# linchaobao/EPPM

Hardware: AMD Instinct MI355X
Metric: Mflow-vectors/sec (higher is better)
Workload: dtype f32; 1 GPU; single 1024x436 Sintel-shape synthetic pair per step, full 3-level pyramid, patch_r=9, default defs.h parameters; 1 rank(s), independent pairs; inputs: RGBA planes resident in HBM before the timed region; outputs: interleaved float2 flow left in HBM (the PCIe-inclusive window of the reference API -- host RGB in, host u/v out -- is `host_boundary`, with --full); inputs=device-resident RGBA, outputs=device-resident float2 flow, pairs_in_flight_per_gpu=24, pairs_per_launch=8, contexts_in_flight=3, width=1024, height=436

## Files before the change

### eppm_amd/_lib.py

```python
import ctypes as C
import os

from .build import lib_path


class EppmError(RuntimeError):
    pass


class CParams(C.Structure):
    _fields_ = [("patch_r", C.c_int), ("num_iter", C.c_int), ("search_range", C.c_int), ("num_guess", C.c_int),
                ("seg_len", C.c_int), ("wmf_iters", C.c_int), ("seed", C.c_ulonglong), ("propagation", C.c_int),
                ("levels", C.c_int)]


class CTrackParams(C.Structure):
    _fields_ = [("spacing", C.c_int), ("min_eig", C.c_int64), ("fb_alpha", C.c_float), ("fb_beta", C.c_float), ("mb_alpha", C.c_float),
                ("mb_beta", C.c_float), ("capacity", C.c_int)]


class CTrackCounts(C.Structure):
    _fields_ = [("live", C.c_int), ("ended", C.c_int), ("seeded", C.c_int), ("dropped", C.c_int), ("frame", C.c_int), ("next_id", C.c_int)]

    def as_dict(self):
        return {k: int(getattr(self, k)) for k, _ in self._fields_}


_lib = None

SYMBOLS = [
    "eppm_default_params", "eppm_create", "eppm_create_batch", "eppm_batch_size", "eppm_batch_set_images", "eppm_batch_set_images_device",
    "eppm_batch_compute", "eppm_batch_compute_device", "eppm_batch_compute_end", "eppm_batch_get_plane", "eppm_destroy", "eppm_set_stream", "eppm_set_images", "eppm_set_images_device",
    "eppm_compute", "eppm_compute_begin", "eppm_compute_end", "eppm_compute_device", "eppm_synchronize", "eppm_num_levels", "eppm_level_dims", "eppm_get_plane",
    "eppm_stage_times", "eppm_clear_stage_times", "eppm_enable_stage_timing", "eppm_last_error", "eppm_version",
    "eppm_device_count", "eppm_set_device", "eppm_malloc_device", "eppm_malloc_pitched", "eppm_free_device",
    "eppm_memcpy_h2d", "eppm_memcpy_d2h", "eppm_memcpy2d_h2d", "eppm_memcpy2d_d2h", "eppm_memset_device",
    "eppm_device_synchronize", "eppm_device_mem_info", "eppm_device_pci_bus_id", "eppm_bind_thread_to_device", "eppm_release_cached_memory", "eppm_set_launcher_stream", "eppm_set_launcher_params", "eppm_launcher_status",
    "baoCudaPatchMatchMultiscalePrepare", "baoCudaCensusTransform", "baoCudaPatchMatch", "baoCudaLeftRightCheck",
    "baoCudaOutlierRemoval", "baoCudaWeightedMedianFilter", "baoCudaFillHole", "baoCudaNNF2Flow", "baoCudaBLF_C2F",
    "baoCudaBLFCostFilterRefine", "baoCudaFlowSmoothing", "eppm_flow_to_color", "eppm_compute_color",
    "eppm_pm_rng_create", "eppm_pm_rng_reset", "eppm_pm_rng_destroy", "eppm_pm_rng_block_states", "eppm_pm_gen_rand_field",
    "eppm_pm_cost_field", "eppm_pm_seg_propagate", "eppm_pm_jump_propagate", "eppm_pm_parallel_propagate", "eppm_pm_random_search", "eppm_gauss_filter_rgba", "eppm_resize_rgba",
    "eppm_resize_flow",
    "eppm_host_register", "eppm_host_unregister", "eppm_host_is_registered", "eppm_host_alloc", "eppm_host_free",
    "eppm_compute_begin_into", "eppm_batch_compute_begin_into",
    "eppm_load_ppm", "eppm_ppm_size", "eppm_save_flo", "eppm_load_flo", "eppm_flo_size", "eppm_flow_error",
    "eppm_flow_error_border", "eppm_flow_error_percentage", "eppm_flow_cutoff", "eppm_flow_to_color_host",
    "eppm_compute_bidirectional", "eppm_compute_bidirectional_device", "eppm_batch_compute_bidirectional", "eppm_set_occlusion_params",
    "eppm_fb_occlusion", "eppm_fb_occlusion_host",
    "eppm_interpolate", "eppm_interpolate_device", "eppm_batch_interpolate", "eppm_interpolate_frames", "eppm_interpolate_host",
    "eppm_track_default_params", "eppm_track_capacity", "eppm_tracker_create", "eppm_tracker_destroy", "eppm_track_step",
    "eppm_track_step_frames", "eppm_tracker_get", "eppm_tracker_get_ended", "eppm_tracker_set", "eppm_track_step_host", "eppm_track_seeds_host",
]


TEST_SYMBOLS = ["eppm_test_set_option", "eppm_probe_c2f_window", "eppm_probe_fast_exp", "eppm_probe_div_const", "eppm_probe_delta_table"]

_variant = None


def select_library(variant):
    global _variant
    if _lib is not None and variant != _variant:
        raise EppmError("select_library: a library is loaded already")
    _variant = variant


def lib():
    global _lib
    if _lib is None:
        path = lib_path(_variant)
        if not os.path.exists(path):
            raise EppmError(f"{path} is missing: run eppm_amd.build() (hipcc --offload-arch=gfx950); there is no CPU fallback")
        L = C.CDLL(path)
        L.eppm_last_error.restype = C.c_char_p
        L.eppm_version.restype = C.c_char_p
        _lib = L
    return _lib


def check(status, what=""):
    if status != 0:
        raise EppmError(f"{what}: status {status}: {lib().eppm_last_error().decode()}")


def check_launcher(what=""):
    check(lib().eppm_launcher_status(), what)
```

### eppm_amd/csrc/context.cpp

```cpp
#include "api_internal.h"
#include "interp.h"

using namespace eppm;


struct StageEv { const char* name; hipEvent_t a, b; };

struct eppm_ctx {
    int device = 0;
    hipStream_t stream = nullptr;
    bool own_stream = false;
    int opt_sweep_spec = -1, opt_no_split = 0;
    eppm_params prm;
    int h = 0, w = 0, nl = 0;
    int npairs = 1, n_active = 1;
    char* slab = nullptr;
    size_t stride = 0;
    int H[kMaxLevels], W[kMaxLevels];
    size_t ipitch[kMaxLevels], cpitch[kMaxLevels];
    uint32_t *raw1 = nullptr, *raw2 = nullptr;
    size_t raw_pitch = 0;
    uint32_t *img1[kMaxLevels] = {}, *img2[kMaxLevels] = {}, *tmpu[kMaxLevels] = {};
    uint8_t *cen1[kMaxLevels] = {}, *cen2[kMaxLevels] = {};
    void *pk1[kMaxLevels] = {}, *pk2[kMaxLevels] = {};
// ... 139 lines not shown
}

static int ctx_alloc(eppm_ctx* c)
{
    const int h = c->h, w = c->w;
    size_t off = 0;
    auto take = [&](size_t bytes) { const size_t o = off; off = (off + bytes + 255) & ~(size_t)255; return o; };
    auto pitch_of = [](size_t row_bytes) { return (row_bytes + 255) & ~(size_t)255; };
    struct Fix { void** dst; size_t off; };
    std::vector<Fix> fix;
    auto plane = [&](void** dst, size_t bytes) { fix.push_back(Fix{dst, take(bytes)}); };
    c->raw_pitch = pitch_of((size_t)w * 4);
    plane((void**)&c->raw1, c->raw_pitch * h);
    plane((void**)&c->raw2, c->raw_pitch * h);
    for (int i = 0; i < c->nl; i++) {
        c->ipitch[i] = pitch_of((size_t)c->W[i] * 4);
        c->cpitch[i] = pitch_of((size_t)c->W[i]);
        const size_t n = (size_t)c->W[i] * c->H[i];
        plane((void**)&c->img1[i], c->ipitch[i] * c->H[i]);
        plane((void**)&c->img2[i], c->ipitch[i] * c->H[i]);
        plane((void**)&c->tmpu[i], c->ipitch[i] * c->H[i]);
        plane(&c->pk1[i], n * 16);
        plane(&c->pk2[i], n * 16);
        plane((void**)&c->pc1[i], n * 4);
        plane((void**)&c->pc2[i], n * 4);
        plane((void**)&c->cen1[i], c->cpitch[i] * c->H[i]);
        plane((void**)&c->cen2[i], c->cpitch[i] * c->H[i]);
        plane((void**)&c->flow[i], n * 8);
        plane((void**)&c->flow_tmp[i], n * 8);
        if (i < c->nl - 1 && c2f_refine_wants_split(c->W[i], c->H[i], c->prm.patch_r, 1, c->opt_no_split != 0)) plane((void**)&c->c2f_cost9[i], n * 36 * 4);
    }
    const int L = c->nl - 1;
    const size_t n2 = (size_t)c->W[L] * c->H[L];
#ifdef EPPM_TOL
    c->pp_pad = (c->prm.patch_r + 2) & ~1;
    c->pp_pitch = parity_pitch(c->W[L], c->pp_pad);
    plane((void**)&c->pp1, (size_t)2 * c->H[L] * c->pp_pitch * 4);
    plane((void**)&c->pp2, (size_t)2 * c->H[L] * c->pp_pitch * 4);
#endif
    plane((void**)&c->nnf1, n2 * 4);
    plane((void**)&c->nnf2, n2 * 4);
    plane((void**)&c->nnf_tmp, n2 * 4);
    plane((void**)&c->nnf_tmp2, n2 * 4);
    plane((void**)&c->cost1, n2 * 4);
    plane((void**)&c->cost2, n2 * 4);
    plane((void**)&c->spec1, n2 * 4 * 4);
    plane((void**)&c->spec2, n2 * 4 * 4);
    plane((void**)&c->scand1, n2 * 4 * 4);
    plane((void**)&c->scand2, n2 * 4 * 4);
    plane((void**)&c->wl1, pm_worklist_words(c->W[L], c->H[L], c->prm.seg_len) * 4);
    plane((void**)&c->wl2, pm_worklist_words(c->W[L], c->H[L], c->prm.seg_len) * 4);
    plane((void**)&c->seed1, n2 * 4 * 4);
    plane((void**)&c->seed2, n2 * 4 * 4);
    plane((void**)&c->wmf_ws, wmf_workspace_words(c->W[L], c->H[L], c->prm.wmf_iters) * 4);
    plane((void**)&c->d_rgb, (size_t)h * w * 3 * 2);
    plane((void**)&c->d_color, (size_t)h * w * 4);
    plane((void**)&c->d_uv, (size_t)h * w * 8);
    CHK(rng_create(&c->rng, c->W[L], c->H[L], c->prm, false));
    const size_t rng_bytes = (size_t)c->rng->gx * c->rng->gy * 64 * 6 * 4;
    for (int k = 0; k < 2; k++)
        for (int q = 0; q < 2; q++) plane((void**)&c->rng->work[k][q], rng_bytes);
    c->stride = (off + 4095) & ~(size_t)4095;
    c->slab_bytes = c->stride * c->npairs;
    {
        const hipError_t e = cache_alloc((void**)&c->slab, c->slab_bytes, false, c->device);
        if (e != hipSuccess) { (void)hipGetLastError(); return set_err(EPPM_ERR_HIP, "hipMalloc of %zu bytes (%d slab(s)) failed: %s", c->slab_bytes, c->npairs, hipGetErrorString(e)); }
    }
    for (const Fix& f : fix) *f.dst = c->slab + f.off;
    CHK(shared_luts(c->device, c->prm.patch_r, &c->lut_pm, &c->lut_wmf, &c->lut_blf));
    c->out_u.assign(c->npairs, nullptr);
    c->out_v.assign(c->npairs, nullptr);
    return EPPM_OK;
// ... 744 lines not shown
        pitch = (size_t)w * esz;
        pstride = c->bwd_stride;
    }
    else return set_err(EPPM_ERR_ARG, "eppm_get_plane: unknown plane '%s' at level %d", name, level);
    if (dst_bytes < (size_t)w * h * esz) return set_err(EPPM_ERR_ARG, "eppm_get_plane: dst too small");
    HIPCHK(hipMemcpy2D(dst, (size_t)w * esz, (const char*)src + (size_t)pair * pstride, pitch, (size_t)w * esz, h, hipMemcpyDeviceToHost));
    return EPPM_OK;
}

extern "C" int eppm_get_plane(eppm_ctx* c, const char* name, int level, void* dst, size_t dst_bytes)
{
    return eppm_batch_get_plane(c, 0, name, level, dst, dst_bytes);
}

extern "C" int eppm_compute_color(eppm_ctx* c, uint8_t* rgb, size_t row_stride, float max_disp_x, float max_disp_y)
{
    if (!c || !rgb) return set_err(EPPM_ERR_ARG, "eppm_compute_color: NULL argument");
    if (!c->have_flow) return set_err(EPPM_ERR_STATE, "eppm_compute_color: no flow computed yet");
    if (row_stride < (size_t)c->w * 3) return set_err(EPPM_ERR_ARG, "eppm_compute_color: row_stride %zu < 3*w", row_stride);
    HIPCHK(hipSetDevice(c->device));
    const size_t n = (size_t)c->h * c->w;
    if (!c->h_color) HIPCHK(hipHostMalloc((void**)&c->h_color, n * 4, hipHostMallocDefault));
    launch_flow_to_color(c->d_color, c->flow[0], c->h, c->w, max_disp_x, max_disp_y, c->stream);
    HIPCHK(hipMemcpyAsync(c->h_color, c->d_color, n * 4, hipMemcpyDeviceToHost, c->stream));
    HIPCHK(hipStreamSynchronize(c->stream));
    for (int y = 0; y < c->h; y++)
        for (int x = 0; x < c->w; x++) {
            const uint32_t p = c->h_color[(size_t)y * c->w + x];
            uint8_t* o = rgb + (size_t)y * row_stride + (size_t)x * 3;
            o[0] = (uint8_t)(p & 0xff); o[1] = (uint8_t)((p >> 8) & 0xff); o[2] = (uint8_t)((p >> 16) & 0xff);
        }
    return EPPM_OK;
}
```

### eppm_amd/csrc/eppm_device.cuh

```cuda
#pragma once

#include <hip/hip_runtime.h>
#include <stdint.h>
#include <float.h>
#include <type_traits>

#include "eppm_internal.h"

namespace eppm {

template <class T>
__device__ __forceinline__ T* pair_ptr(T* p, size_t stride, unsigned pair)
{
    using Byte = typename std::conditional<std::is_const<T>::value, const char, char>::type;
    return reinterpret_cast<T*>(reinterpret_cast<Byte*>(p) + stride * pair);
}
template <class T>
__device__ __forceinline__ T* pair_ptr_opt(T* p, size_t stride, unsigned pair)
{
    return p ? pair_ptr(p, stride, pair) : p;
}

constexpr float kLambdaAd2 = 0.1f * 0.1f;
constexpr float kPmSigR2 = 0.1f * 0.1f;
// ... 34 lines not shown
__device__ __forceinline__ float unorm8(float c) { constexpr DivConst d = make_div_const(255.0f); return div_const(c, d); }

struct rgbf { float x, y, z; };

__device__ __forceinline__ rgbf unpack_rgb(uint32_t p)
{
    rgbf r;
    r.x = unorm8((float)(p & 0xffu));
    r.y = unorm8((float)((p >> 8) & 0xffu));
    r.z = unorm8((float)((p >> 16) & 0xffu));
    return r;
}

__device__ __forceinline__ int iclamp(int v, int lo, int hi) { return min(max(v, lo), hi); }
__device__ __forceinline__ int med3i(int v, int lo, int hi)
{
    int r;
    asm("v_med3_i32 %0, %1, %2, %3" : "=v"(r) : "v"(v), "v"(lo), "v"(hi));
    return r;
}

__device__ __forceinline__ float max_abs_diff(const rgbf a, const rgbf b)
{
    return fmaxf(fmaxf(fabsf(a.x - b.x), fabsf(a.y - b.y)), fabsf(a.z - b.z));
}

struct Planes {
    const float4* pk1;
    const float4* pk2;
    int w, h;
    int pitch;
};

#ifndef EPPM_TOL
#ifndef EPPM_CENSUS_POPCNT
#define EPPM_CENSUS_POPCNT 1
#endif
__device__ __forceinline__ float4 make_texel(uint32_t rgba, uint32_t census)
{
    const rgbf c = unpack_rgb(rgba);
    return make_float4(c.x, c.y, c.z, __uint_as_float(EPPM_CENSUS_POPCNT ? (census & 0xffu) * 0x01010101u : (census & 0xffu) << 2));
}
__device__ __forceinline__ float census_cost(const float* __restrict__ cnx, uint32_t w1, uint32_t w2)
{
    return *reinterpret_cast<const float*>(reinterpret_cast<const char*>(cnx) + (EPPM_CENSUS_POPCNT ? (uint32_t)__builtin_popcount(w1 ^ w2) : (w1 ^ w2)));
}
#else
constexpr unsigned kTolScale = 4u;
__device__ __forceinline__ float4 make_texel(uint32_t rgba, uint32_t census)
{
    return make_float4(__uint_as_float((rgba & 0xffu) * kTolScale), __uint_as_float(((rgba >> 8) & 0xffu) * kTolScale),
                       __uint_as_float(((rgba >> 16) & 0xffu) * kTolScale), __uint_as_float((census & 0xffu) * 0x01010101u));
}
#endif
__device__ __forceinline__ float one_minus_fast_exp(float x) { return 1 - fast_exp(x); }

struct DeltaTab {
    int t1[256];
    float t2[kDeltaSlots];
};
#ifndef EPPM_DELTA_PATCH
#define EPPM_DELTA_PATCH 1
#endif
#ifndef EPPM_DELTA_BLF
#define EPPM_DELTA_BLF 1
#endif
typedef const __attribute__((address_space(3))) float lds_cfloat;
typedef const __attribute__((address_space(3))) int lds_cint;
__device__ __forceinline__ uint32_t lds_addr(const void* p) { return (uint32_t)(uintptr_t)(const __attribute__((address_space(3))) void*)p; }
__device__ __forceinline__ float delta_lookup(const DeltaTab& D, float d)
{
    const uint32_t a1 = __float_as_uint(__builtin_fmaf(d, __uint_as_float(1020u), __uint_as_float(lds_addr(D.t1))));
    const uint32_t a2 = (__float_as_uint(d) << 2) + (uint32_t)*reinterpret_cast<lds_cint*>(a1);
    return *reinterpret_cast<lds_cfloat*>(a2);
}
__device__ __forceinline__ float delta_lookup_off(const DeltaTab& D, float d)
{
    const uint32_t o1 = __float_as_uint(d * __uint_as_float(1020u));
// ... 70 lines not shown
    float cn[16];
};
__device__ __forceinline__ uint32_t linf_off(const rgbf a, const rgbf b) { return __float_as_uint(max_abs_diff(a, b)); }
__device__ __forceinline__ float tol_at(const float* __restrict__ t, uint32_t byte_off)
{
    return *reinterpret_cast<const float*>(reinterpret_cast<const char*>(t) + byte_off);
}
__device__ __forceinline__ float tol_cost(const TolTables& T, const rgbf p1, const rgbf p2, uint32_t w1, uint32_t w2)
{
    return tol_at(T.td, linf_off(p1, p2)) + tol_at(T.cn, (uint32_t)__builtin_popcount(w1 ^ w2));
}
constexpr float kTolExpC = (float)(1.4426950408889634 / (255.0 * 255.0 * (double)kPmSigR2) / (double)(kTolScale * kTolScale));
constexpr float kTolWeightBias = 24.0f;
__device__ __forceinline__ float tol_exp_arg(uint32_t off4k, float lsrc)
{
    const float kf = __uint_as_float(off4k) * 0x1p100f;
    return __builtin_fmaf(kf * kf, -kTolExpC * 0x1p98f, lsrc);
}
__device__ __forceinline__ rgbf tol_scale_centre(const rgbf c) { return rgbf{c.x * 0x1p100f, c.y * 0x1p100f, c.z * 0x1p100f}; }
__device__ __forceinline__ float tol_exp_arg_scaled(const rgbf cs, const rgbf p, float lsrc)
{
    const float kf = fmaxf(fmaxf(fabsf(__builtin_fmaf(p.x, 0x1p100f, -cs.x)), fabsf(__builtin_fmaf(p.y, 0x1p100f, -cs.y))), fabsf(__builtin_fmaf(p.z, 0x1p100f, -cs.z)));
    return __builtin_fmaf(kf * kf, -kTolExpC * 0x1p98f, lsrc);
}
__device__ __forceinline__ float4 unpack_texel(uint32_t w, uint32_t two)
{
    uint32_t r, g, b;
    asm("v_lshlrev_b32_sdwa %0, %1, %2 dst_sel:DWORD dst_unused:UNUSED_PAD src0_sel:DWORD src1_sel:BYTE_0" : "=v"(r) : "v"(two), "v"(w));
    asm("v_lshlrev_b32_sdwa %0, %1, %2 dst_sel:DWORD dst_unused:UNUSED_PAD src0_sel:DWORD src1_sel:BYTE_1" : "=v"(g) : "v"(two), "v"(w));
    asm("v_lshlrev_b32_sdwa %0, %1, %2 dst_sel:DWORD dst_unused:UNUSED_PAD src0_sel:DWORD src1_sel:BYTE_2" : "=v"(b) : "v"(two), "v"(w));
    static_assert(kTolScale == 4u, "the shift above");
    return make_float4(__uint_as_float(r), __uint_as_float(g), __uint_as_float(b), __uint_as_float(__builtin_amdgcn_perm(w, w, 0x03030303u)));
}
typedef uint32_t u32x4 __attribute__((ext_vector_type(4)));
typedef uint32_t u32x2 __attribute__((ext_vector_type(2)));
__device__ __forceinline__ void patch_terms(const float4 q1, const float4 q2, const rgbf c1, const rgbf c2, float gsp,
                                            const TolTables& T, float& cost_term, float& weight_term)
{
    const rgbf p1 = texel_rgb(q1);
    const rgbf p2 = texel_rgb(q2);
    cost_term = tol_cost(T, p1, p2, __float_as_uint(q1.w), __float_as_uint(q2.w));
    weight_term = (tol_at(T.ta, linf_off(c1, p1)) * gsp) * tol_at(T.ta, linf_off(c2, p2));
}
__device__ __forceinline__ void patch_accum(float& cost_sum, float& weight_sum, float cost_term, float weight_term)
{
    cost_sum = __builtin_fmaf(cost_term, weight_term, cost_sum);
    weight_sum += weight_term;
}
#endif

template <class TAB>
__device__ __forceinline__ void patch_sample(const Planes& P, const rgbf c1, const rgbf c2, int sx1, int sy1, int sx2,
                                             int sy2, float gsp, const TAB& cnx, float& cost_term,
                                             float& weight_term)
{
    const float4 q1 = tex_px(P.pk1, P.pitch, P.w, P.h, sx1, sy1);
    const float4 q2 = tex_px(P.pk2, P.pitch, P.w, P.h, sx2, sy2);
    patch_terms(q1, q2, c1, c2, gsp, cnx, cost_term, weight_term);
}

__host__ __device__ constexpr int tol_chunk(int R) { return R == 17 ? 6 : (R + 2) / 2; }
struct PatchSum {
    float cs = 0.0f, ws = 0.0f;
#ifdef EPPM_TOL
    float cc = 0.0f, cw = 0.0f;
    __device__ __forceinline__ void add(float cost_term, float weight_term) { patch_accum(cc, cw, cost_term, weight_term); }
    __device__ __forceinline__ void flush() { cs += cc; ws += cw; cc = 0.0f; cw = 0.0f; }
#else
// ... 154 lines not shown
```

### eppm_amd/csrc/eppm_internal.h

```cpp
#pragma once

#include <hip/hip_runtime.h>
#include <stddef.h>
#include <stdint.h>

#include "../../include/eppm.h"

namespace eppm {

constexpr int kMaxLevels = 8;
constexpr int kNumLevels = 3;
constexpr int kBlock = 16;
constexpr int kMaxS = 32;
constexpr int kWmfRadius = 4;
constexpr int kBlfRadius = 10;
constexpr int kDeltaSlots = 800;

struct Batch {
    int n;
    size_t stride;
};
constexpr Batch kOnePair = {1, 0};

struct PlanesH {
// ... 35 lines not shown
    int32_t* scand = nullptr;
    uint32_t* wl = nullptr;
    int16_t* seed = nullptr;
    uint32_t* rng_work;
    uint32_t* rng_work_next;
};
struct PmBatch {
    PmProblem p[2];
    int n;
    int cpitch, npitch;
    int npairs = 1;
    size_t stride = 0;
    size_t cache_plane = 0;
    int wl_units = 0;
    int sweep_seq = 0;
    size_t seed_plane = 0;
    int merged_it = 0;
    int seg_len = 0, nseg_row = 0, nseg_col = 0;
};
int pm_worklist_units(int w, int h, int seg_len);
inline size_t pm_worklist_words(int w, int h, int seg_len) { return 16 + 10 * (size_t)pm_worklist_units(w, h, seg_len); }
struct PmRngDev {
    const uint32_t* init_tab;
    const uint32_t* iter_tab;
    const uint32_t* skip_mat;
    uint32_t skip_weyl;
    int per_lane;
    int gx, gy;
    const int16_t* rand_tab = nullptr;
};
void launch_pm_rand_table(const PmRngDev& rng, uint32_t* work, int16_t* tab, int G, hipStream_t s);
void launch_pm_init_field(const PmBatch& b, const PmRngDev& rng, hipStream_t s);
void launch_pm_cost_field(const PmBatch& b, const float* lut, int R, hipStream_t s);
bool launch_pm_sweep(PmBatch& b, const float* lut, int R, int seg_len, int dir, hipStream_t s, bool speculative = false);
bool launch_pm_sweeps_merged(PmBatch& b, const float* lut, int R, int seg_len, int iteration, hipStream_t s);
void launch_pm_jump(const PmBatch& b, const float* lut, int R, int step, hipStream_t s);
void launch_pm_neighbor(const PmBatch& b, const float* lut, int R, hipStream_t s);
void launch_pm_random_search(const PmBatch& b, const PmRngDev& rng, const float* lut, int R, int search_range, int num_guess,
                             hipStream_t s);

void launch_lr_check(int16_t* nnf1, float* cost1, const int16_t* nnf2, int w, int h, int cost_pitch, int nnf_pitch, hipStream_t s, Batch bt = kOnePair);
void launch_outlier(int16_t* nnf_out, float* cost, const int16_t* nnf_in, int w, int h, int cost_pitch, int nnf_pitch, hipStream_t s, Batch bt = kOnePair);
size_t wmf_workspace_words(int w, int h, int num_iter);
int16_t* launch_wmf(int16_t* buf_a, int16_t* buf_b, const uint32_t* img, int ipitch, int w, int h, int nnf_pitch,
                    const float* wmf_lut, int num_iter, int only_occlusion, uint32_t* ws, hipStream_t s, Batch bt = kOnePair);
void launch_fill_holes(int16_t* nnf_out, const int16_t* nnf_in, const uint32_t* img, int ipitch, int w, int h, int nnf_pitch,
                       hipStream_t s, Batch bt = kOnePair);
void launch_nnf2flow(float* flow, int flow_pitch, const int16_t* nnf, int nnf_pitch, int w, int h, hipStream_t s, Batch bt = kOnePair);

void launch_resize_flow(float* out, int outH, int outW, const float* in, int h, int w, float ratio, float post_scale, hipStream_t s, Batch bt = kOnePair);
void launch_mul_scalar(float* flow, float scale, int h, int w, hipStream_t s);
bool c2f_refine_wants_split(int w, int h, int R, int npairs = 1, bool no_split = false);
bool c2f_window_span(int R, int* span_x, int* span_y);
void launch_c2f_refine(const PlanesH& P, float* flow, const float* lut, int R, float* cost9, hipStream_t s, Batch bt = kOnePair, bool no_split = false);
void launch_flow_blf(float* out, const float* in, const uint32_t* img, int ipitch, int w, int h, int flow_pitch,
                     const float* blf_lut, hipStream_t s, Batch bt = kOnePair);

void launch_split_flow(float* uv, const float* flow, int n, hipStream_t s, Batch bt = kOnePair);

void launch_fb_occlusion(uint8_t* occ1, uint8_t* occ2, const float* fwd, size_t fwd_stride, const float* bwd, size_t bwd_stride, int h, int w,
                         float alpha, float beta, int npairs, int ndir, hipStream_t s);

constexpr int kInterpChunk = 4;
struct InterpArgs {
    const uint8_t* img1;
    const uint8_t* img2;
// ... 26 lines not shown
    struct {
        int spacing;
        long long min_eig;
        float fb_alpha, fb_beta, mb_alpha, mb_beta;
    } p;
    int cap, ncells, ncx;
    float* npos;
    uint8_t* stat;
    TrackRec* ended;
    int32_t* ended_reason;
    uint8_t* cov;
    uint8_t* flags;
    int32_t *blk_s, *blk_e;
    int32_t* blk_c;
    int32_t* cnt;
};
struct TrackIn {
    const uint8_t* img1;
    const uint8_t* img2;
    size_t pitch;
    const float* fwd;
    const float* bwd;
    int h, w;
};
void launch_track_seed0(const TrackDev& d, const TrackIn& in, TrackRec* cur, hipStream_t s);
void launch_track_advance(const TrackDev& d, const TrackIn& in, const TrackRec* cur, hipStream_t s);
void launch_track_seed(const TrackDev& d, const TrackIn& in, hipStream_t s);
void launch_track_compact(const TrackDev& d, const TrackIn& in, const TrackRec* cur, TrackRec* next, hipStream_t s);

void launch_flow_to_color(uint32_t* rgba, const float* flow, int h, int w, float max_disp_x, float max_disp_y, hipStream_t s, Batch bt = kOnePair);

void launch_probe_delta(const float* x, float* y, int n, const float* delta_tab, hipStream_t s);
void launch_probe(const float* x, float* y, int n, int which, hipStream_t s);

struct XorwowState { uint32_t v[5]; uint32_t d; };
void xorwow_init(XorwowState* s, unsigned long long seed, unsigned long long subsequence);
uint32_t xorwow_next(XorwowState* s);
void xorwow_skip_matrix(unsigned long long n, uint32_t* out);

}
```

### eppm_amd/csrc/k_patchmatch.hip

```cpp
#include "eppm_device.cuh"
#include "eppm_internal.h"

#ifndef EPPM_LPC9
#ifdef EPPM_TOL
#define EPPM_LPC9 32
#else
#define EPPM_LPC9 16
#endif
#endif
#ifndef EPPM_SWEEP_GB
#define EPPM_SWEEP_GB 7
#endif
#ifndef EPPM_LPC17
#define EPPM_LPC17 64
#endif
#ifndef EPPM_LPC9_SPEC
#ifdef EPPM_TOL
#define EPPM_LPC9_SPEC 32
#else
#define EPPM_LPC9_SPEC 16
#endif
#endif
#ifndef EPPM_LPC17_SPEC
#define EPPM_LPC17_SPEC 64
// ... 81 lines not shown
{
    __shared__ EPPM_LUT_ALIGN PatchLut L;
    load_patch_lut(L, lut, R, threadIdx.y * kBlock + threadIdx.x, 256);
    __syncthreads();
    const PmProblem pr = pm_problem(B, blockIdx.z);
    const Planes P = to_dev(pr.P);
    const int x = blockIdx.x * kBlock + threadIdx.x, y = blockIdx.y * kBlock + threadIdx.y;
    if (x >= P.w || y >= P.h) return;
    const int dx = pr.nnf[(y * B.npitch + x) * 2], dy = pr.nnf[(y * B.npitch + x) * 2 + 1];
    pr.cost[y * B.cpitch + x] = patch_dist(P, L, R, x, y, dx, dy);
}


template <int RT> struct SearchLut { using type = PatchLutT<RT + 1>; };
template <> struct SearchLut<0> { using type = PatchLut; };

__device__ __forceinline__ float patch_dist_any(const Planes& P, const PatchLut& L, int R, int x1, int y1, int x2, int y2) { return patch_dist(P, L, R, x1, y1, x2, y2); }
template <int M> __device__ __forceinline__ float patch_dist_any(const Planes&, const PatchLutT<M>&, int, int, int, int, int) { return 0.0f; }

#define EPPM_PM_PRAGMA_(x) _Pragma(#x)
#define EPPM_PM_UNROLL(n) EPPM_PM_PRAGMA_(unroll n)
template <int RT, int PK = 0, class LUT>
__device__ __forceinline__ float search_patch_dist(const Planes& P, const LUT& L, int R, const float4* __restrict__ s_src, int TW,
                                                   int tx, int ty, int x1, int y1, int x2, int y2, const PlanesH& PH)
{
    if (RT == 0) return patch_dist_any(P, L, R, x1, y1, x2, y2);
    constexpr int S = RT + 1;
    const int pitch16 = P.pitch << 4;
    const rgbf c1 = texel_rgb(s_src[(ty + RT) * TW + tx + RT]);
    const rgbf c2 = texel_rgb(texel_at(P.pk2, texel_off(pitch16, P.w, P.h, x2, y2)));
    PatchSum sum;
    constexpr int CS = tol_chunk(RT);
    static_assert(S % CS == 0, "whole chunks per row");
#ifdef EPPM_TOL
    if constexpr (PK == 2) {
        static_assert(S % 4 == 2, "a row = whole dwordx4 gathers + one dwordx2");
        const __amdgpu_buffer_rsrc_t rs = __builtin_amdgcn_make_buffer_rsrc(const_cast<uint32_t*>(PH.pp2), 0, 2 * P.h * PH.pp_pitch * 4, 0x00020000);
        const int xp = x2 - RT + PH.pp_pad;
        const int rb = ((xp & 1) * P.h) * PH.pp_pitch + (xp >> 1);
        uint32_t two = 2u;
        asm volatile("" : "+v"(two));
#pragma unroll 2
        for (int ii = 0; ii < S; ii++) {
            const int ro = (rb + iclamp(y2 + 2 * ii - RT, 0, P.h - 1) * PH.pp_pitch) * 4;
            const float4* __restrict__ srow = s_src + (ty + 2 * ii) * TW + tx;
            uint32_t wq[S];
#pragma unroll
            for (int g = 0; g < S / 4; g++) {
                const u32x4 v = __builtin_amdgcn_raw_buffer_load_b128(rs, ro + 16 * g, 0, 0);
                wq[4 * g] = v.x; wq[4 * g + 1] = v.y; wq[4 * g + 2] = v.z; wq[4 * g + 3] = v.w;
            }
            { const u32x2 v = __builtin_amdgcn_raw_buffer_load_b64(rs, ro + 4 * (S - 2), 0, 0); wq[S - 2] = v.x; wq[S - 1] = v.y; }
#ifdef EPPM_SEARCH_TERM_UNROLL
            constexpr int TU = EPPM_SEARCH_TERM_UNROLL;
#else
            constexpr int TU = (S % 5 == 0) ? 5 : (S % 9 == 0) ? 9 : S;
#endif
EPPM_PM_UNROLL((TU))
            for (int jj = 0; jj < S; jj++) {
                float ct, wt;
                patch_terms(srow[2 * jj], unpack_texel(wq[jj], two), c1, c2, L.gsp[ii * S + jj], L.tab(), ct, wt);
                sum.add(ct, wt);
                if ((jj + 1) % CS == 0) sum.flush();
            }
        }
        return sum.result();
    }
#endif
    const uint32_t* __restrict__ pc2 = PH.pc2;
    for (int ii = 0; ii < S; ii++) {
        const int i = 2 * ii - RT;
        const unsigned r2 = __umul24((unsigned)iclamp(y2 + i, 0, P.h - 1), (unsigned)pitch16);
        const float4* __restrict__ srow = s_src + (ty + 2 * ii) * TW + tx;
        for (int j0 = 0; j0 < S; j0 += 5) {
            float4 q1[5], q2[5];
            uint32_t w2[PK == 1 ? 5 : 1];
#pragma unroll
            for (int k = 0; k < 5; k++) {
                const int jj = min(j0 + k, S - 1);
                q1[k] = srow[2 * jj];
                const unsigned o2 = r2 + ((unsigned)iclamp(x2 + 2 * jj - RT, 0, P.w - 1) << 4);
                if (PK == 1) w2[k] = *reinterpret_cast<const uint32_t*>(reinterpret_cast<const char*>(pc2) + (o2 >> 2));
                else q2[k] = texel_at(P.pk2, o2);
            }
#pragma unroll
            for (int k = 0; k < 5; k++) {
                if (j0 + k < S) {
                    float ct, wt;
                    if (PK == 1) q2[k] = make_texel(w2[k], w2[k] >> 24);
                    patch_terms(q1[k], q2[k], c1, c2, L.gsp[ii * S + j0 + k], L.tab(), ct, wt);
                    sum.add(ct, wt);
                    if ((j0 + k + 1) % CS == 0) sum.flush();
                }
            }
        }
    }
    return sum.result();
}

template <int RT, int PK = 0>
__global__ __launch_bounds__(256) void k_pm_cost_field_tile(PmBatch B, const float* __restrict__ lut, int R)
{
    using LUT = typename SearchLut<RT>::type;
    constexpr int TW = kBlock + 2 * RT;
    __shared__ float4 s_src[TW * TW];
    __shared__ EPPM_LUT_ALIGN LUT L;
    const int tid = threadIdx.y * kBlock + threadIdx.x;
    load_patch_lut(L, lut, R, tid, 256);
    const PmProblem pr = pm_problem(B, blockIdx.z);
    const Planes P = to_dev(pr.P);
    const int x0 = blockIdx.x * kBlock - RT, y0 = blockIdx.y * kBlock - RT;
    for (int t = tid; t < TW * TW; t += 256) {
        const int sy = iclamp(y0 + t / TW, 0, P.h - 1), sx = iclamp(x0 + t % TW, 0, P.w - 1);
        s_src[t] = P.pk1[(unsigned)(sy * P.pitch + sx)];
    }
    __syncthreads();
    const int x = blockIdx.x * kBlock + threadIdx.x, y = blockIdx.y * kBlock + threadIdx.y;
    if (x >= P.w || y >= P.h) return;
    const int dx = pr.nnf[(y * B.npitch + x) * 2], dy = pr.nnf[(y * B.npitch + x) * 2 + 1];
    pr.cost[y * B.cpitch + x] = search_patch_dist<RT, PK>(P, L, R, s_src, TW, threadIdx.x, threadIdx.y, x, y, dx, dy, pr.P);
}

static bool pm_has_parity(const PmBatch& b)
{
#ifdef EPPM_TOL
    return b.p[0].P.pp2 && (b.n < 2 || b.p[1].P.pp2);
#else
    return false;
#endif
}

void launch_pm_cost_field(const PmBatch& b, const float* lut, int R, hipStream_t s)
{
    const int w = b.p[0].P.w, h = b.p[0].P.h;
    dim3 grid((w + kBlock - 1) / kBlock, (h + kBlock - 1) / kBlock, b.n * b.npairs), block(kBlock, kBlock);
#ifndef EPPM_COST_FIELD_TILE
#define EPPM_COST_FIELD_TILE 1
#endif
    if (EPPM_COST_FIELD_TILE && R == 9 && pm_has_parity(b)) hipLaunchKernelGGL((k_pm_cost_field_tile<9, 2>), grid, block, 0, s, b, lut, R);
    else if (EPPM_COST_FIELD_TILE && R == 17 && pm_has_parity(b)) hipLaunchKernelGGL((k_pm_cost_field_tile<17, 2>), grid, block, 0, s, b, lut, R);
    else if (EPPM_COST_FIELD_TILE && R == 9) hipLaunchKernelGGL(k_pm_cost_field_tile<9>, grid, block, 0, s, b, lut, R);
    else if (EPPM_COST_FIELD_TILE && R == 17) hipLaunchKernelGGL(k_pm_cost_field_tile<17>, grid, block, 0, s, b, lut, R);
    else hipLaunchKernelGGL(k_pm_cost_field, grid, block, 0, s, b, lut, R);
}

template <int LPC>
__device__ __forceinline__ float dpp_prev_lane(float v)
{
    if (LPC == 4) return __int_as_float(__builtin_amdgcn_update_dpp(0, __float_as_int(v), 0x93 , 0xf, 0xf, false));
    if (LPC == 16) return __int_as_float(__builtin_amdgcn_update_dpp(0, __float_as_int(v), 0x121 , 0xf, 0xf, false));
    return __int_as_float(__builtin_amdgcn_update_dpp(0, __float_as_int(v), 0x138 , 0xf, 0xf, false));
}

template <int R, int LPC>
__host__ __device__ constexpr int coop_chunk()
{
#ifdef EPPM_TOL
    return tol_chunk(R);
#else
    return ((R + 1) * (R + 1) + LPC - 1) / LPC;
#endif
}
template <int LPC, int CH, int NS, int NL>
__device__ __forceinline__ void coop_chain_sum(const float (&tc)[CH], const float (&tw)[CH], float& ac, float& aw)
{
#ifdef EPPM_TOL
    float pc = 0.0f, pw = 0.0f;
#pragma unroll
    for (int q = 0; q < CH; q++) patch_accum(pc, pw, tc[q], tw[q]);
#pragma unroll
    for (int ln = 0; ln < NL; ln++) {
        if (ln > 0) { ac = dpp_prev_lane<LPC>(ac); aw = dpp_prev_lane<LPC>(aw); }
        ac += pc; aw += pw;
// ... 531 lines not shown
        const int sidx = IS_ROW ? (line * B.npitch + start) : (start * B.npitch + line);
        px = nnf[sidx * 2];
        py = nnf[sidx * 2 + 1];
    }
    __syncthreads();
    for (int s = 0; s < L_; s++) {
        if (active && s < count) {
            const int x = IS_ROW ? i : line, y = IS_ROW ? line : i;
            const int nidx = y * B.npitch + x, cidx = y * B.cpitch + x;
            const float cur_best = cost[cidx];
            if (IS_ROW) px = REVERSE ? max(px - 1, 0) : min(px + 1, P.w - 1);
            else        py = REVERSE ? max(py - 1, 0) : min(py + 1, P.h - 1);
            const bool same = (px == nnf[nidx * 2]) && (py == nnf[nidx * 2 + 1]);
            const float cv = same ? cur_best : patch_dist(P, L, R, x, y, px, py);
            if (cv < cur_best) {
                nnf[nidx * 2] = (int16_t)px;
                nnf[nidx * 2 + 1] = (int16_t)py;
                cost[cidx] = cv;
            } else {
                px = nnf[nidx * 2];
                py = nnf[nidx * 2 + 1];
            }
            i += step;
        }
        if (!REVERSE && s == 0) __syncthreads();
    }
}

template <int RT>
static void launch_sweep_spec(const PmBatch& b, const float* lut, int R, int dir, int seg_len, int nseg, hipStream_t s)
{
    const int w = b.p[0].P.w, h = b.p[0].P.h, gx = (w + kBlock - 1) / kBlock, gy = (h + kBlock - 1) / kBlock;
    dim3 grid(gx * gy * (b.n * b.npairs)), block(256);
    if (pm_has_parity(b)) {
        switch (dir) {
            case 0: hipLaunchKernelGGL((k_pm_sweep_spec<RT, true, false, 2>), grid, block, 0, s, b, lut, R, gx, seg_len, nseg); break;
            case 1: hipLaunchKernelGGL((k_pm_sweep_spec<RT, false, false, 2>), grid, block, 0, s, b, lut, R, gx, seg_len, nseg); break;
            case 2: hipLaunchKernelGGL((k_pm_sweep_spec<RT, true, true, 2>), grid, block, 0, s, b, lut, R, gx, seg_len, nseg); break;
            default: hipLaunchKernelGGL((k_pm_sweep_spec<RT, false, true, 2>), grid, block, 0, s, b, lut, R, gx, seg_len, nseg); break;
        }
        return;
    }
    switch (dir) {
        case 0: hipLaunchKernelGGL((k_pm_sweep_spec<RT, true, false>), grid, block, 0, s, b, lut, R, gx, seg_len, nseg); break;
        case 1: hipLaunchKernelGGL((k_pm_sweep_spec<RT, false, false>), grid, block, 0, s, b, lut, R, gx, seg_len, nseg); break;
        case 2: hipLaunchKernelGGL((k_pm_sweep_spec<RT, true, true>), grid, block, 0, s, b, lut, R, gx, seg_len, nseg); break;
        default: hipLaunchKernelGGL((k_pm_sweep_spec<RT, false, true>), grid, block, 0, s, b, lut, R, gx, seg_len, nseg); break;
    }
}
int pm_worklist_units(int w, int h, int seg_len)
{
    const int ur = h * (((w + seg_len - 1) / seg_len + 1) / 2), uc = w * (((h + seg_len - 1) / seg_len + 1) / 2);
    return ur > uc ? ur : uc;
}
template <int R, int LPC>
static void launch_sweep_b(const PmBatch& b, const float* lut, int seg_len, int dir, int nseg, int lines, hipStream_t s)
{
    constexpr int CPB = 256 / LPC;
    const int nseg_pad = (nseg + 1) & ~1;
    const int wgs = (lines * nseg_pad + CPB - 1) / CPB;
    dim3 grid(wgs * (b.n * b.npairs)), block(256);
    switch (dir) {
        case 0: hipLaunchKernelGGL((k_pm_sweep<R, LPC, true, false, false, true>), grid, block, 0, s, b, lut, seg_len, nseg, nseg_pad, 0); break;
        case 1: hipLaunchKernelGGL((k_pm_sweep<R, LPC, false, false, false, true>), grid, block, 0, s, b, lut, seg_len, nseg, nseg_pad, 0); break;
        case 2: hipLaunchKernelGGL((k_pm_sweep<R, LPC, true, true, false, true>), grid, block, 0, s, b, lut, seg_len, nseg, nseg_pad, 0); break;
        default: hipLaunchKernelGGL((k_pm_sweep<R, LPC, false, true, false, true>), grid, block, 0, s, b, lut, seg_len, nseg, nseg_pad, 0); break;
    }
// ... 73 lines not shown
        default: hipLaunchKernelGGL((k_pm_seg_propagate<false, true>), grid, block, 0, s, b, lut, R, seg_len, nseg, lpb); break;
    }
    return false;
}

template <int R, int LPC>
static void launch_sweep_merged(const PmBatch& b, const float* lut, int seg_len, int dir, hipStream_t s)
{
    const PlanesH& P = b.p[0].P;
    const bool is_row = (dir == 0 || dir == 2);
    const int len = is_row ? P.w : P.h, lines = is_row ? P.h : P.w;
    const int nseg = (len + seg_len - 1) / seg_len, nseg_pad = (nseg + 1) & ~1;
    constexpr int CPB = 256 / LPC;
    const int wgs = (lines * nseg_pad + CPB - 1) / CPB;
    dim3 grid(wgs * (b.n * b.npairs)), block(256);
    switch (dir) {
        case 0: hipLaunchKernelGGL((k_pm_sweep<R, LPC, true, false, false, false, true, true>), grid, block, 0, s, b, lut, seg_len, nseg, nseg_pad, 0); break;
        case 1: hipLaunchKernelGGL((k_pm_sweep<R, LPC, false, false, false, false, true, true>), grid, block, 0, s, b, lut, seg_len, nseg, nseg_pad, 0); break;
        case 2: hipLaunchKernelGGL((k_pm_sweep<R, LPC, true, true, false, false, true, true>), grid, block, 0, s, b, lut, seg_len, nseg, nseg_pad, 0); break;
        default: hipLaunchKernelGGL((k_pm_sweep<R, LPC, false, true, false, false, true, true>), grid, block, 0, s, b, lut, seg_len, nseg, nseg_pad, 0); break;
    }
}
bool launch_pm_sweeps_merged(PmBatch& b, const float* lut, int R, int seg_len, int iteration, hipStream_t s)
{
    for (int k = 0; k < b.n; k++)
        if (!b.p[k].seed || !b.p[k].wl || !b.p[k].spec || !b.p[k].scand) return false;
    if (!(R == 9 || R == 17) || seg_len > kSpecMaxSteps || seg_len < 1) return false;
    const int w = b.p[0].P.w, h = b.p[0].P.h, gx = (w + kBlock - 1) / kBlock, gy = (h + kBlock - 1) / kBlock;
    b.merged_it = iteration;
    b.seg_len = seg_len;
    b.nseg_row = (w + seg_len - 1) / seg_len;
    b.nseg_col = (h + seg_len - 1) / seg_len;
    dim3 grid(gx * gy * (b.n * b.npairs)), block(256);
    if (R == 9 && pm_has_parity(b)) hipLaunchKernelGGL((k_pm_spec_all<9, 2>), grid, block, 0, s, b, lut, R, gx);
    else if (pm_has_parity(b)) hipLaunchKernelGGL((k_pm_spec_all<17, 2>), grid, block, 0, s, b, lut, R, gx);
    else if (R == 9) hipLaunchKernelGGL(k_pm_spec_all<9>, grid, block, 0, s, b, lut, R, gx);
    else hipLaunchKernelGGL(k_pm_spec_all<17>, grid, block, 0, s, b, lut, R, gx);
    for (int dir = 0; dir < 4; dir++) {
        if (R == 9) launch_sweep_merged<9, EPPM_LPC9_SPEC>(b, lut, seg_len, dir, s);
        else launch_sweep_merged<17, EPPM_LPC17_SPEC>(b, lut, seg_len, dir, s);
        b.sweep_seq++;
    }
    return true;
}

template <bool NEIGHBOR>
__global__ __launch_bounds__(256) void k_pm_jump(PmBatch B, const float* __restrict__ lut, int R, int step)
{
    __shared__ EPPM_LUT_ALIGN PatchLut L;
    __shared__ float s_cost[4][64];
    __shared__ int s_cand[4][64];
    const PmProblem pr = pm_problem(B, blockIdx.z);
    const int tid = threadIdx.x, lane = tid & 63, k = tid >> 6;
    load_patch_lut(L, lut, R, tid, 256);
    __syncthreads();
    const Planes P = to_dev(pr.P);
    const int x = blockIdx.x * kBlock + (lane & 15), y = blockIdx.y * 4 + (lane >> 4);
    const bool inimg = (x < P.w && y < P.h);
    const int nidx = y * B.npitch + x, cidx = y * B.cpitch + x;
    int bx = 0, by = 0;
    float cv = FLT_MAX;
    int cand = -1;
    if (inimg) {
        bx = pr.nnf[nidx * 2]; by = pr.nnf[nidx * 2 + 1];
        if (NEIGHBOR) {
            const int nx = iclamp(x + ((k == 2) ? -1 : (k == 3) ? 1 : 0), 0, P.w - 1);
            const int ny = iclamp(y + ((k == 0) ? -1 : (k == 1) ? 1 : 0), 0, P.h - 1);
            const int dx = pr.nnf[(ny * B.npitch + nx) * 2], dy = pr.nnf[(ny * B.npitch + nx) * 2 + 1];
// ... 165 lines not shown
    if (inimg) {
        float cv = INFINITY;
        if (evaluate) {
            cv = search_patch_dist<RT, PK>(P, L, R, s_src, TW, lane & 15, lane >> 4, x, y, gx, gy, pr.P);
        }
        s_cost[k][lane] = cv;
    }
    __syncthreads();
    if (k == 0 && inimg) {
        float best_cost = pr.cost[cidx];
        for (int g = 0; g < G; g++) {
            const float cv = s_cost[g][lane];
            if (cv < best_cost) {
                const int e = s_guess[g][lane];
                bx = (int)(int16_t)(e & 0xffff); by = e >> 16; best_cost = cv;
            }
        }
        pr.nnf[nidx * 2] = (int16_t)bx;
        pr.nnf[nidx * 2 + 1] = (int16_t)by;
        pr.cost[cidx] = best_cost;
    }
}

void launch_pm_random_search(const PmBatch& b, const PmRngDev& rng, const float* lut, int R, int search_range, int num_guess,
                             hipStream_t s)
{
    dim3 grid(rng.gx * rng.gy * 4 * b.n * b.npairs), block(64 * (num_guess + 1));
    if (rng.rand_tab && (R == 9 || R == 17)) {
        dim3 blockt(64 * num_guess);
        const bool have_pc_t = b.p[0].P.pc2 && (b.n < 2 || b.p[1].P.pc2);
#ifndef EPPM_SEARCH_HALF_BELOW_WGS
#define EPPM_SEARCH_HALF_BELOW_WGS 1024
#endif
        if (pm_has_parity(b)) {
            if (R == 9 && (int)grid.x < EPPM_SEARCH_HALF_BELOW_WGS)
                hipLaunchKernelGGL((k_pm_random_search<9, 2, true, 2>), dim3(grid.x * 2), dim3(32 * num_guess), 0, s, b, rng, lut, R, search_range, num_guess);
            else if (R == 9) hipLaunchKernelGGL((k_pm_random_search<9, 2, true>), grid, blockt, 0, s, b, rng, lut, R, search_range, num_guess);
            else hipLaunchKernelGGL((k_pm_random_search<17, 2, true>), grid, blockt, 0, s, b, rng, lut, R, search_range, num_guess);
            return;
        }
        if (R == 9 && (int)grid.x < EPPM_SEARCH_HALF_BELOW_WGS) {
            hipLaunchKernelGGL((k_pm_random_search<9, 0, true, 2>), dim3(grid.x * 2), dim3(32 * num_guess), 0, s, b, rng, lut, R, search_range, num_guess);
            return;
        }
        if (R == 9) hipLaunchKernelGGL((k_pm_random_search<9, 0, true>), grid, blockt, 0, s, b, rng, lut, R, search_range, num_guess);
        else if (have_pc_t) hipLaunchKernelGGL((k_pm_random_search<17, 1, true>), grid, blockt, 0, s, b, rng, lut, R, search_range, num_guess);
        else hipLaunchKernelGGL((k_pm_random_search<17, 0, true>), grid, blockt, 0, s, b, rng, lut, R, search_range, num_guess);
        return;
    }
#ifndef EPPM_SEARCH_PK17
#define EPPM_SEARCH_PK17 1
#endif
    const bool have_pc = b.p[0].P.pc2 && (b.n < 2 || b.p[1].P.pc2);
    if (R == 17 && have_pc && EPPM_SEARCH_PK17) hipLaunchKernelGGL((k_pm_random_search<17, 1>), grid, block, 0, s, b, rng, lut, R, search_range, num_guess);
    else if (R == 9) hipLaunchKernelGGL(k_pm_random_search<9>, grid, block, 0, s, b, rng, lut, R, search_range, num_guess);
    else if (R == 17) hipLaunchKernelGGL(k_pm_random_search<17>, grid, block, 0, s, b, rng, lut, R, search_range, num_guess);
    else hipLaunchKernelGGL(k_pm_random_search<0>, grid, block, 0, s, b, rng, lut, R, search_range, num_guess);
}

}
```

### eppm_amd/csrc/k_probe.hip

```cpp
#include "eppm_device.cuh"
#include "eppm_internal.h"

namespace eppm {

__global__ void k_probe(const float* __restrict__ x, float* __restrict__ y, int n, int which)
{
    const int i = blockIdx.x * blockDim.x + threadIdx.x;
    if (i >= n) return;
    const float v = x[i];
    float r;
    if (which == 0) r = fast_exp(v);
    else if (which == 1) r = div_ad2(v);
    else if (which == 2) r = div_wmf2(v);
    else r = unorm8(v);
    y[i] = r;
}
__global__ __launch_bounds__(256) void k_probe_delta(const float* __restrict__ x, float* __restrict__ y, int n, const float* __restrict__ tab)
{
    __shared__ DeltaTab s_D, s_E;
    load_delta_tab(s_D, tab, threadIdx.x, 256);
    load_delta_tab<false>(s_E, tab, threadIdx.x, 256);
    __syncthreads();
    const int i = blockIdx.x * blockDim.x + threadIdx.x;
    if (i < n) {
        const float a = delta_lookup(s_D, x[i]), b = delta_lookup_off(s_E, x[i]);
        y[i] = (__float_as_uint(a) == __float_as_uint(b)) ? a : __uint_as_float(0x7fc00000u);
    }
}
void launch_probe_delta(const float* x, float* y, int n, const float* tab, hipStream_t s)
{
    hipLaunchKernelGGL(k_probe_delta, dim3((n + 255) / 256), dim3(256), 0, s, x, y, n, tab);
}
void launch_probe(const float* x, float* y, int n, int which, hipStream_t s)
{
    hipLaunchKernelGGL(k_probe, dim3((n + 255) / 256), dim3(256), 0, s, x, y, n, which);
}

}
```

Before: 224.2 Mflow-vectors/s.

## Enable parity-split packed image layout for exact R=9 search and cost field

Extends the parity-plane packed image layout, previously compiled only for the tolerance build, to the exact build when patch_r is 9. The random-search and cost-field kernels then use the PK=2 parity gather path, which reads dwordx4/dwordx2 buffer loads. The speculative sweep path stays on the old layout by default. In exchange it allocates two extra parity planes per context and depends on those planes being filled correctly, and it adds a texel unpack helper plus test probes.

Result: faster. 232.3 Mflow-vectors/s (median of 6 runs) (+3.6%).

```diff
diff --git a/eppm_amd/_lib.py b/eppm_amd/_lib.py
--- a/eppm_amd/_lib.py
+++ b/eppm_amd/_lib.py
@@ -54,7 +54,8 @@
 ]
 
 
-TEST_SYMBOLS = ["eppm_test_set_option", "eppm_probe_c2f_window", "eppm_probe_fast_exp", "eppm_probe_div_const", "eppm_probe_delta_table"]
+TEST_SYMBOLS = ["eppm_test_set_option", "eppm_probe_c2f_window", "eppm_probe_fast_exp", "eppm_probe_div_const", "eppm_probe_delta_table",
+                "eppm_probe_unpack_texel", "eppm_probe_pm_parity"]
 
 _variant = None
 
diff --git a/eppm_amd/csrc/context.cpp b/eppm_amd/csrc/context.cpp
--- a/eppm_amd/csrc/context.cpp
+++ b/eppm_amd/csrc/context.cpp
@@ -195,12 +195,15 @@
     }
     const int L = c->nl - 1;
     const size_t n2 = (size_t)c->W[L] * c->H[L];
-#ifdef EPPM_TOL
-    c->pp_pad = (c->prm.patch_r + 2) & ~1;
-    c->pp_pitch = parity_pitch(c->W[L], c->pp_pad);
-    plane((void**)&c->pp1, (size_t)2 * c->H[L] * c->pp_pitch * 4);
-    plane((void**)&c->pp2, (size_t)2 * c->H[L] * c->pp_pitch * 4);
+#ifndef EPPM_TOL
+    if (c->prm.patch_r == 9)
 #endif
+    {
+        c->pp_pad = (c->prm.patch_r + 2) & ~1;
+        c->pp_pitch = parity_pitch(c->W[L], c->pp_pad);
+        plane((void**)&c->pp1, (size_t)2 * c->H[L] * c->pp_pitch * 4);
+        plane((void**)&c->pp2, (size_t)2 * c->H[L] * c->pp_pitch * 4);
+    }
     plane((void**)&c->nnf1, n2 * 4);
     plane((void**)&c->nnf2, n2 * 4);
     plane((void**)&c->nnf_tmp, n2 * 4);
@@ -1011,3 +1014,14 @@
         }
     return EPPM_OK;
 }
+
+#ifdef EPPM_TEST_HOOKS
+extern "C" int eppm_probe_pm_parity(const eppm_ctx* c, int* pitch, int* pad, int* kernels)
+{
+    if (!c || !pitch || !pad || !kernels) return set_err(EPPM_ERR_ARG, "eppm_probe_pm_parity: NULL argument");
+    *pitch = c->pp1 ? c->pp_pitch : 0;
+    *pad = c->pp1 ? c->pp_pad : 0;
+    *kernels = c->pp1 ? pm_parity_kernels(c->prm.patch_r) : 0;
+    return EPPM_OK;
+}
+#endif
diff --git a/eppm_amd/csrc/eppm_device.cuh b/eppm_amd/csrc/eppm_device.cuh
--- a/eppm_amd/csrc/eppm_device.cuh
+++ b/eppm_amd/csrc/eppm_device.cuh
@@ -90,6 +90,9 @@
     int pitch;
 };
 
+typedef uint32_t u32x4 __attribute__((ext_vector_type(4)));
+typedef uint32_t u32x2 __attribute__((ext_vector_type(2)));
+
 #ifndef EPPM_TOL
 #ifndef EPPM_CENSUS_POPCNT
 #define EPPM_CENSUS_POPCNT 1
@@ -102,6 +105,12 @@
 __device__ __forceinline__ float census_cost(const float* __restrict__ cnx, uint32_t w1, uint32_t w2)
 {
     return *reinterpret_cast<const float*>(reinterpret_cast<const char*>(cnx) + (EPPM_CENSUS_POPCNT ? (uint32_t)__builtin_popcount(w1 ^ w2) : (w1 ^ w2)));
+}
+__device__ __forceinline__ float4 unpack_texel(uint32_t w, uint32_t)
+{
+    static_assert(EPPM_CENSUS_POPCNT, "the census byte replicated into its word (make_texel)");
+    const rgbf c = unpack_rgb(w);
+    return make_float4(c.x, c.y, c.z, __uint_as_float(__builtin_amdgcn_perm(w, w, 0x03030303u)));
 }
 #else
 constexpr unsigned kTolScale = 4u;
@@ -238,8 +247,6 @@
     static_assert(kTolScale == 4u, "the shift above");
     return make_float4(__uint_as_float(r), __uint_as_float(g), __uint_as_float(b), __uint_as_float(__builtin_amdgcn_perm(w, w, 0x03030303u)));
 }
-typedef uint32_t u32x4 __attribute__((ext_vector_type(4)));
-typedef uint32_t u32x2 __attribute__((ext_vector_type(2)));
 __device__ __forceinline__ void patch_terms(const float4 q1, const float4 q2, const rgbf c1, const rgbf c2, float gsp,
                                             const TolTables& T, float& cost_term, float& weight_term)
 {
diff --git a/eppm_amd/csrc/eppm_internal.h b/eppm_amd/csrc/eppm_internal.h
--- a/eppm_amd/csrc/eppm_internal.h
+++ b/eppm_amd/csrc/eppm_internal.h
@@ -91,6 +91,7 @@
 void launch_pm_rand_table(const PmRngDev& rng, uint32_t* work, int16_t* tab, int G, hipStream_t s);
 void launch_pm_init_field(const PmBatch& b, const PmRngDev& rng, hipStream_t s);
 void launch_pm_cost_field(const PmBatch& b, const float* lut, int R, hipStream_t s);
+int pm_parity_kernels(int R);
 bool launch_pm_sweep(PmBatch& b, const float* lut, int R, int seg_len, int dir, hipStream_t s, bool speculative = false);
 bool launch_pm_sweeps_merged(PmBatch& b, const float* lut, int R, int seg_len, int iteration, hipStream_t s);
 void launch_pm_jump(const PmBatch& b, const float* lut, int R, int step, hipStream_t s);
@@ -183,6 +184,7 @@
 
 void launch_probe_delta(const float* x, float* y, int n, const float* delta_tab, hipStream_t s);
 void launch_probe(const float* x, float* y, int n, int which, hipStream_t s);
+void launch_probe_unpack(const uint32_t* w, float* y, int n, hipStream_t s);
 
 struct XorwowState { uint32_t v[5]; uint32_t d; };
 void xorwow_init(XorwowState* s, unsigned long long seed, unsigned long long subsequence);
diff --git a/eppm_amd/csrc/k_patchmatch.hip b/eppm_amd/csrc/k_patchmatch.hip
--- a/eppm_amd/csrc/k_patchmatch.hip
+++ b/eppm_amd/csrc/k_patchmatch.hip
@@ -137,7 +137,6 @@
     PatchSum sum;
     constexpr int CS = tol_chunk(RT);
     static_assert(S % CS == 0, "whole chunks per row");
-#ifdef EPPM_TOL
     if constexpr (PK == 2) {
         static_assert(S % 4 == 2, "a row = whole dwordx4 gathers + one dwordx2");
         const __amdgpu_buffer_rsrc_t rs = __builtin_amdgcn_make_buffer_rsrc(const_cast<uint32_t*>(PH.pp2), 0, 2 * P.h * PH.pp_pitch * 4, 0x00020000);
@@ -171,7 +170,6 @@
         }
         return sum.result();
     }
-#endif
     const uint32_t* __restrict__ pc2 = PH.pc2;
     for (int ii = 0; ii < S; ii++) {
         const int i = 2 * ii - RT;
@@ -226,13 +224,31 @@
     pr.cost[y * B.cpitch + x] = search_patch_dist<RT, PK>(P, L, R, s_src, TW, threadIdx.x, threadIdx.y, x, y, dx, dy, pr.P);
 }
 
-static bool pm_has_parity(const PmBatch& b)
+#ifndef EPPM_PARITY_SEARCH
+#define EPPM_PARITY_SEARCH 1
+#endif
+#ifndef EPPM_PARITY_SPEC
+#define EPPM_PARITY_SPEC 0
+#endif
+#ifndef EPPM_PARITY_COST
+#define EPPM_PARITY_COST 1
+#endif
+static bool pm_parity_adopted(int R, bool exact_adopts)
 {
 #ifdef EPPM_TOL
-    return b.p[0].P.pp2 && (b.n < 2 || b.p[1].P.pp2);
+    (void)exact_adopts;
+    return R == 9 || R == 17;
 #else
-    return false;
-#endif
+    return exact_adopts && R == 9;
+#endif
+}
+static bool pm_has_parity(const PmBatch& b, int R, bool exact_adopts)
+{
+    return pm_parity_adopted(R, exact_adopts) && b.p[0].P.pp2 && (b.n < 2 || b.p[1].P.pp2);
+}
+int pm_parity_kernels(int R)
+{
+    return (pm_parity_adopted(R, EPPM_PARITY_SEARCH) ? 1 : 0) | (pm_parity_adopted(R, EPPM_PARITY_SPEC) ? 2 : 0) | (pm_parity_adopted(R, EPPM_PARITY_COST) ? 4 : 0);
 }
 
 void launch_pm_cost_field(const PmBatch& b, const float* lut, int R, hipStream_t s)
@@ -242,8 +258,8 @@
 #ifndef EPPM_COST_FIELD_TILE
 #define EPPM_COST_FIELD_TILE 1
 #endif
-    if (EPPM_COST_FIELD_TILE && R == 9 && pm_has_parity(b)) hipLaunchKernelGGL((k_pm_cost_field_tile<9, 2>), grid, block, 0, s, b, lut, R);
-    else if (EPPM_COST_FIELD_TILE && R == 17 && pm_has_parity(b)) hipLaunchKernelGGL((k_pm_cost_field_tile<17, 2>), grid, block, 0, s, b, lut, R);
+    if (EPPM_COST_FIELD_TILE && R == 9 && pm_has_parity(b, R, EPPM_PARITY_COST)) hipLaunchKernelGGL((k_pm_cost_field_tile<9, 2>), grid, block, 0, s, b, lut, R);
+    else if (EPPM_COST_FIELD_TILE && R == 17 && pm_has_parity(b, R, EPPM_PARITY_COST)) hipLaunchKernelGGL((k_pm_cost_field_tile<17, 2>), grid, block, 0, s, b, lut, R);
     else if (EPPM_COST_FIELD_TILE && R == 9) hipLaunchKernelGGL(k_pm_cost_field_tile<9>, grid, block, 0, s, b, lut, R);
     else if (EPPM_COST_FIELD_TILE && R == 17) hipLaunchKernelGGL(k_pm_cost_field_tile<17>, grid, block, 0, s, b, lut, R);
     else hipLaunchKernelGGL(k_pm_cost_field, grid, block, 0, s, b, lut, R);
@@ -841,7 +857,7 @@
 {
     const int w = b.p[0].P.w, h = b.p[0].P.h, gx = (w + kBlock - 1) / kBlock, gy = (h + kBlock - 1) / kBlock;
     dim3 grid(gx * gy * (b.n * b.npairs)), block(256);
-    if (pm_has_parity(b)) {
+    if (pm_has_parity(b, RT, EPPM_PARITY_SPEC)) {
         switch (dir) {
             case 0: hipLaunchKernelGGL((k_pm_sweep_spec<RT, true, false, 2>), grid, block, 0, s, b, lut, R, gx, seg_len, nseg); break;
             case 1: hipLaunchKernelGGL((k_pm_sweep_spec<RT, false, false, 2>), grid, block, 0, s, b, lut, R, gx, seg_len, nseg); break;
@@ -981,8 +997,8 @@
     b.nseg_row = (w + seg_len - 1) / seg_len;
     b.nseg_col = (h + seg_len - 1) / seg_len;
     dim3 grid(gx * gy * (b.n * b.npairs)), block(256);
-    if (R == 9 && pm_has_parity(b)) hipLaunchKernelGGL((k_pm_spec_all<9, 2>), grid, block, 0, s, b, lut, R, gx);
-    else if (pm_has_parity(b)) hipLaunchKernelGGL((k_pm_spec_all<17, 2>), grid, block, 0, s, b, lut, R, gx);
+    if (R == 9 && pm_has_parity(b, R, EPPM_PARITY_SPEC)) hipLaunchKernelGGL((k_pm_spec_all<9, 2>), grid, block, 0, s, b, lut, R, gx);
+    else if (pm_has_parity(b, R, EPPM_PARITY_SPEC)) hipLaunchKernelGGL((k_pm_spec_all<17, 2>), grid, block, 0, s, b, lut, R, gx);
     else if (R == 9) hipLaunchKernelGGL(k_pm_spec_all<9>, grid, block, 0, s, b, lut, R, gx);
     else hipLaunchKernelGGL(k_pm_spec_all<17>, grid, block, 0, s, b, lut, R, gx);
     for (int dir = 0; dir < 4; dir++) {
@@ -1214,7 +1230,7 @@
 #ifndef EPPM_SEARCH_HALF_BELOW_WGS
 #define EPPM_SEARCH_HALF_BELOW_WGS 1024
 #endif
-        if (pm_has_parity(b)) {
+        if (pm_has_parity(b, R, EPPM_PARITY_SEARCH)) {
             if (R == 9 && (int)grid.x < EPPM_SEARCH_HALF_BELOW_WGS)
                 hipLaunchKernelGGL((k_pm_random_search<9, 2, true, 2>), dim3(grid.x * 2), dim3(32 * num_guess), 0, s, b, rng, lut, R, search_range, num_guess);
             else if (R == 9) hipLaunchKernelGGL((k_pm_random_search<9, 2, true>), grid, blockt, 0, s, b, rng, lut, R, search_range, num_guess);
diff --git a/eppm_amd/csrc/k_probe.hip b/eppm_amd/csrc/k_probe.hip
--- a/eppm_amd/csrc/k_probe.hip
+++ b/eppm_amd/csrc/k_probe.hip
@@ -31,6 +31,18 @@
 {
     hipLaunchKernelGGL(k_probe_delta, dim3((n + 255) / 256), dim3(256), 0, s, x, y, n, tab);
 }
+__global__ __launch_bounds__(256) void k_probe_unpack(const uint32_t* __restrict__ w, float4* __restrict__ y, int n)
+{
+    const int i = blockIdx.x * blockDim.x + threadIdx.x;
+    if (i >= n) return;
+    const uint32_t v = w[i];
+    y[2 * i] = unpack_texel(v, 2u);
+    y[2 * i + 1] = make_texel(v, v >> 24);
+}
+void launch_probe_unpack(const uint32_t* w, float* y, int n, hipStream_t s)
+{
+    hipLaunchKernelGGL(k_probe_unpack, dim3((n + 255) / 256), dim3(256), 0, s, w, (float4*)y, n);
+}
 void launch_probe(const float* x, float* y, int n, int which, hipStream_t s)
 {
     hipLaunchKernelGGL(k_probe, dim3((n + 255) / 256), dim3(256), 0, s, x, y, n, which);
```
